# Lcressot/fhe-string-bounty

Measured on AMD Instinct MI355X. Metric: PBS/sec (whole node), higher is better.
Workload: dtype f64

## Files before the change

### fhe-string-bounty_amd/csrc/engine.h

```cpp
#pragma once
#include <hip/hip_runtime.h>
#include <stdint.h>

#include <map>
#include <mutex>
#include <string>
#include <vector>

#include "../../include/fhestr.h"

#define FHESTR_KERNEL_REVISION "r04.2"

namespace fhe {

inline uint32_t n_ggsw(const fhe_params_t& p) {
    return p.grouping_factor > 1 ? p.n / p.grouping_factor * (1u << p.grouping_factor) : p.n;
}
inline uint64_t multi_bit_key_bit(const uint64_t* group_bits, uint32_t g, uint32_t sel) {
    uint64_t prod = 1;
    for (uint32_t b = 0; b < g; b++) prod *= group_bits[b] ^ (((sel >> (g - 1 - b)) & 1) ^ 1);
    return prod;
}

void aes128_round_keys(const uint8_t key[16], uint8_t rk[11][16]);
const uint8_t* aes_sbox();

extern thread_local std::string g_last_error;
int fail(const std::string& msg);

struct BrVariant;

uint64_t fill_accumulator(const fhe_params_t& p, const uint64_t* table, std::vector<uint64_t>& acc);
void fill_accumulator_torus(const fhe_params_t& p, const uint64_t* box_values, std::vector<uint64_t>& acc);

struct EngineEnv {
    int log2_points = 0;
    int wide_fair = -1;
    int keep_busy = -1;
    int overlap_streams = -1;
    int ks_mfma = -1;
    int ks_chunks = -1;
    int cluster_mode = -2;
    int cluster_spin_limit = -1;
    int multibit_combine_max = -1;
    int cluster_test_fault = -1;
    int dense_per_cu = -1;
    int cluster_fallback = -1;
    static EngineEnv read();
};

struct Engine {
    std::recursive_mutex mu;
    fhe_params_t p{};
    int device = 0;
    hipStream_t stream = nullptr;
    hipStream_t own_stream = nullptr;
    std::map<std::vector<uint64_t>, uint32_t> lut_dedup;
    hipEvent_t ev[3] = {nullptr, nullptr, nullptr};
    std::vector<hipEvent_t> ring;
    size_t ring_used = 0;
    const BrVariant* variant = nullptr;
    const BrVariant* variant_large = nullptr;
    int cu_count = 256;
    int pipeline = 0;
    hipStream_t ks_stream = nullptr;
    hipEvent_t pipe_ev[5] = {nullptr, nullptr, nullptr, nullptr, nullptr};
    hipEvent_t pipe_input_ready = nullptr;
    const void* pipe_out[2] = {nullptr, nullptr};
    size_t pipe_out_bytes[2] = {0, 0};
    static constexpr int OVL_MAX = 4;
    int ovl_streams = 2;
    uint32_t wide_fair_shift = 13;
    uint32_t dense_per_cu = 2;
    bool keep_busy = false;
    hipStream_t ovl_stream[OVL_MAX] = {nullptr, nullptr, nullptr, nullptr};
    hipEvent_t ovl_done[OVL_MAX] = {nullptr, nullptr, nullptr, nullptr};
    struct ByteRange { const char* lo; const char* hi; };
    std::vector<ByteRange> ovl_ins[OVL_MAX], ovl_outs[OVL_MAX];
    uint64_t* ovl_small[OVL_MAX] = {nullptr, nullptr, nullptr, nullptr};
    size_t ovl_cap_small[OVL_MAX] = {0, 0, 0, 0};
    int8_t* ovl_digits[OVL_MAX] = {nullptr, nullptr, nullptr, nullptr};
    size_t ovl_cap_digits[OVL_MAX] = {0, 0, 0, 0};
    int sync_all_streams();
    void end_pipeline_run();
    uint64_t pipe_calls = 0;
    int shadow_fit = -1;
    uint32_t multibit_combine_max = 64;

    uint32_t* d_ksk_packed = nullptr;
    uint64_t* d_ksk_rowsum = nullptr;
    int8_t* d_ksk_mfma = nullptr;
    int8_t* d_ks_digits = nullptr;
    size_t cap_ks_digits = 0;
    bool ks_mfma_enabled = true;
    double* d_fbsk = nullptr;
    double* d_fbsk_dense = nullptr;
    uint64_t* d_luts = nullptr;
    size_t luts_cap = 0;
    uint32_t n_luts = 0;

    uint64_t *d_in = nullptr, *d_small = nullptr, *d_small2 = nullptr, *d_out = nullptr, *d_pool = nullptr;
    uint32_t* d_idx = nullptr;
    uint32_t* d_slot_exp = nullptr;
    size_t multibit_workspace_cap = 0;
    void* d_meta = nullptr;
    uint64_t* d_compact = nullptr;
    size_t cap_compact = 0;
    void* d_ws = nullptr;
    size_t cap_ws = 0;
    void* d_cluster_ws = nullptr;
    size_t cap_cluster_ws = 0;
    void* d_cluster_ctl = nullptr;
    bool cluster_unchecked = false;
    uint32_t cluster_last = 0;
    bool cluster_fallback = true;
    uint32_t cluster_fallbacks = 0;
    uint32_t cluster_last_error = 0;
    int cluster_mode = -1;
    uint32_t cluster_max_batch = 0xFFFFFFFFu;
    uint32_t ks_chunks_override = 0;
    int xcd_per_cu = -1;
    uint32_t xcd_auto_max = 16;
    uint32_t cluster_spin_limit = 1u << 22;
    uint32_t cluster_test_fault = 0;
    int cluster_check();
    size_t cap_in = 0, cap_small = 0, cap_small2 = 0, cap_out = 0, cap_idx = 0, cap_pool = 0, cap_meta = 0;

    static int create(const fhe_params_t& p, int device, Engine** out);
    ~Engine();
    int use();
    int set_variant(int logR);
    int allow_rotate_lds();
    int load_keys(const uint64_t* bsk_std, const uint64_t* ksk);
    int load_seeded_keys(const uint8_t ksk_seed[16], const uint64_t* ksk_bodies, const uint8_t bsk_seed[16], const uint64_t* bsk_bodies,
                         uint64_t* bsk_std_out, uint64_t* ksk_out);
    int expand_seeded_lwe(const uint8_t* seeds, const uint64_t* bodies, uint32_t count, uint64_t* d_out, uint64_t* host_out);
    int expand_compact_list(const uint64_t* list, uint32_t count, uint64_t* d_out, uint64_t* host_out);
    int expand_compact_list_dev(const uint64_t* d_list, uint32_t count, uint64_t* d_out);
    int generate_keys(const uint64_t* glwe_sk, const uint64_t* small_sk, const uint8_t seed[32],
                      uint64_t* bsk_std_out, uint64_t* ksk_out);
    int install_keys(uint64_t* d_ksk_std, uint64_t* d_bsk_std);
    int convert_polys(const uint64_t* d_std, double* d_out, uint32_t n_polys);
    int cluster_settle(const uint64_t* d_sm, const uint32_t* d_lut_idx, uint64_t* d_big, uint32_t count);
    int probe_slot_exponents();
    uint64_t fill_accumulator(const uint64_t* table, std::vector<uint64_t>& acc) const { return fhe::fill_accumulator(p, table, acc); }
    int lut_upload_dedup(const std::vector<uint64_t>& acc, uint32_t* id);
    int set_stream(hipStream_t s, bool use_own);
    int lut_upload(const uint64_t* acc, uint32_t* id);
    int lut_download(uint32_t id, uint64_t* acc);
    int ensure_batch(uint32_t count);
    int check_lut_idx(const uint32_t* lut_idx, uint32_t count) const;

    int launch_keyswitch(const uint64_t* d_big, uint64_t* d_sm, uint32_t count, hipStream_t on = nullptr, bool shadow = false, int digits_slot = 0);
    int launch_blind_rotate(const uint64_t* d_sm, const uint32_t* d_lut_idx, uint64_t* d_big, uint32_t count, hipStream_t on = nullptr, bool two_per_cu = false,
                            bool one_workgroup_only = false);
    bool shadow_keyswitch_fits();
    int ks_pbs_dev(const uint64_t* d_big_in, const uint32_t* d_lut_idx, uint64_t* d_big_out, uint32_t count, bool allow_pipeline = false);
    int ks_pbs_host(const uint64_t* in, const uint32_t* lut_idx, uint64_t* out, uint32_t count);
    int keyswitch_host(const uint64_t* in, uint64_t* out_small, uint32_t count);
    int pbs_host(const uint64_t* in_small, const uint32_t* lut_idx, uint64_t* out, uint32_t count);
    int pbs_ks_host(const uint64_t* in_small, const uint32_t* lut_idx, uint64_t* out_small, uint32_t count);
    int lincomb_dev(const uint64_t* d_pool, const uint32_t* d_off, const uint32_t* d_src,
                    const int32_t* d_coeff, const uint64_t* d_cst, uint64_t* d_out, uint32_t jobs);
// ... 26 lines not shown
```

### fhe-string-bounty_amd/csrc/engine.hip

```cpp
#include "engine.h"

#include <algorithm>
#include <cmath>
#include <cstdio>
#include <cstdlib>
#include <cstring>
#include <string>

#include "keygen_kernels.hip.h"
#include "lwe_kernels.hip.h"
#include "ks_mfma_kernels.hip.h"
#include "pbs_kernels.hip.h"
#include "pbs_dense_kernels.hip.h"
#include "pbs_large_kernels.hip.h"
#include "pbs_cluster_kernels.hip.h"
#include "pbs_xcd_kernels.hip.h"
#include "pbs_multibit_kernels.hip.h"
#include "pbs_seq_kernels.hip.h"
#include "seeded_kernels.hip.h"
#include "compact_kernels.hip.h"

namespace fhe {

thread_local std::string g_last_error;
// ... 166 lines not shown
                                  : reinterpret_cast<const void*>(&multibit_combine_generic_kernel<3>);
    v.combined_bytes = (size_t)v.L * v.k1 * v.k1 * ((size_t)1 << (v.logN - 1)) * 16;
    return v;
}
template <int LOGN, int LOGR, int K1, int L>
BrVariant make_multibit_generic_variant(int G) {
    return make_multibit_two_kernel_variant<&blind_rotate_kernel<LOGN, LOGR, K1, L, true>>(make_variant<LOGN, LOGR, K1, L>(), G);
}
template <int LOGN, int K1, int L>
BrVariant make_multibit_seq_variant(int G) {
    return make_multibit_two_kernel_variant<&blind_rotate_seq_kernel<LOGN, K1, L, true>>(make_seq_variant<LOGN, K1, L>(), G);
}

static const std::vector<BrVariant>& variants() {
    static const std::vector<BrVariant> v = {
        make_variant<11, 2, 2, 1>(), make_variant<11, 3, 2, 1>(), make_variant<11, 4, 2, 1>(),
        make_wide_variant<11, 2, 2, 1>(), make_wide_variant<11, 3, 2, 1>(),
        make_multibit_variant<11, 2, 2, 2>(),
        make_multibit_variant<11, 2, 2, 3>(),
        make_multibit_generic_variant<9, 2, 4, 1>(2), make_multibit_generic_variant<9, 2, 4, 1>(3),
        make_multibit_seq_variant<13, 2, 2>(2), make_multibit_seq_variant<13, 2, 2>(3),
        make_multibit_generic_variant<8, 2, 2, 2>(2), make_multibit_generic_variant<8, 2, 2, 2>(3),
        make_multibit_generic_variant<7, 2, 3, 1>(2), make_multibit_generic_variant<7, 2, 3, 1>(3),
        make_variant<10, 2, 3, 1>(), make_variant<10, 3, 3, 1>(), make_wide_variant<10, 2, 3, 1>(),
        make_variant<9, 2, 4, 1>(),
        make_variant<8, 2, 2, 2>(), make_variant<7, 2, 3, 1>(),
        make_wide_variant<8, 2, 2, 2>(), make_wide_variant<7, 2, 3, 1>(),
        make_variant<8, 2, 6, 1>(),
        make_variant<9, 2, 3, 2>(),
        make_wide_variant<12, 2, 2, 1>(), make_wide_variant<12, 2, 2, 2>(),
        make_seq_variant<13, 2, 1>(), make_seq_variant<13, 2, 2>(),
        make_large_variant<14, 2, 2>(),
        make_large_variant<15, 2, 2>(),
        make_large_variant<14, 2, 3>(), make_large_variant<15, 2, 3>(),
    };
    return v;
}

static const BrVariant* find_variant(const fhe_params_t& p, int selector) {
    int logN = 0;
    while ((1u << logN) < p.N) logN++;
    const int logR = selector & 15;
    const bool wide = (selector & 16) != 0;
    const int grouping = p.grouping_factor > 1 ? (int)p.grouping_factor : 1;
    for (const auto& v : variants())
        if (v.logN == logN && v.k1 == (int)p.k + 1 && v.L == (int)p.pbs_level && v.grouping == grouping &&
            (selector == 0 || (v.logR == logR && v.wide == wide)))
            return &v;
    return nullptr;
}

struct BrVariantPair { const BrVariant *small, *large; };
static BrVariantPair find_variant_pair(const fhe_params_t& p, int selector) {
    const BrVariant* v = find_variant(p, selector);
    const BrVariant* w = v && selector == 0 ? find_variant(p, v->logR | 16) : nullptr;
    return {v, w ? w : v};
}

static size_t rotate_lds(const BrVariant* v, const fhe_params_t& p) { return v->lds_bytes + (size_t)p.n * v->lds_per_n; }

int params_supported(const fhe_params_t& p, int selector) {
    if ((p.N & (p.N - 1)) || p.N < 128) return fail("polynomial size must be a power of two >= 128");
    if (p.pbs_base_log < 1 || p.pbs_base_log > 31 || p.pbs_base_log * p.pbs_level > (p.pbs_level >= 3 ? 62u : 31u))
        return fail("unsupported PBS decomposition (base_log * level must be <= 31, or <= 62 with >= 3 levels)");
    if (p.ks_level < 1 || p.ks_base_log < 1 || p.ks_base_log > 7 || p.ks_base_log * p.ks_level > 62)
        return fail("unsupported keyswitch decomposition (base_log 1..7, base_log * level <= 62)");
    if (p.msg_mod * p.carry_mod == 0 || (p.N % (p.msg_mod * p.carry_mod)) != 0)
        return fail("msg_mod * carry_mod must divide N");
    if (p.grouping_factor > 1 && (p.n % p.grouping_factor) != 0) return fail("grouping factor must divide n");
    if (!find_variant(p, selector)) return fail("no blind-rotation kernel instantiated for this (N, k, level, grouping factor)");
    return 0;
}
int params_supported(const fhe_params_t& p) { return params_supported(p, 0); }

EngineEnv EngineEnv::read() {
    EngineEnv v;
    auto num = [](const char* name, int& out) { if (const char* t = getenv(name)) out = atoi(t); };
    num("FHESTR_LOG2_POINTS", v.log2_points);
    num("FHESTR_WIDE_FAIR", v.wide_fair);
    num("FHESTR_DENSE_PER_CU", v.dense_per_cu);
    num("FHESTR_CLUSTER_FALLBACK", v.cluster_fallback);
    num("FHESTR_KEEP_BUSY", v.keep_busy);
    num("FHESTR_OVERLAP_STREAMS", v.overlap_streams);
    num("FHESTR_KS_MFMA", v.ks_mfma);
    num("FHESTR_KS_CHUNKS", v.ks_chunks);
    num("FHESTR_CLUSTER", v.cluster_mode);
    num("FHESTR_CLUSTER_SPIN_LIMIT", v.cluster_spin_limit);
    num("FHESTR_MULTIBIT_COMBINE_MAX", v.multibit_combine_max);
    num("FHESTR_CLUSTER_TEST_FAULT", v.cluster_test_fault);
    return v;
}

int Engine::create(const fhe_params_t& p, int device, Engine** out) {
    const EngineEnv env = EngineEnv::read();
    if (params_supported(p, env.log2_points)) return 1;
    int count = 0;
    HIP_TRY(hipGetDeviceCount(&count));
    if (count <= 0) return fail("no HIP device: libfhestr has no CPU fallback");
    if (device < 0 || device >= count) return fail("bad device index");
    HIP_TRY(hipSetDevice(device));
    Engine* e = new Engine();
    e->p = p;
    e->device = device;
    const BrVariantPair vp = find_variant_pair(p, env.log2_points);
    e->variant = vp.small;
    e->variant_large = vp.large;
    if (env.wide_fair >= 0) e->wide_fair_shift = (uint32_t)std::min(20, env.wide_fair);
    if (env.dense_per_cu >= 0) e->dense_per_cu = (uint32_t)env.dense_per_cu;
    if (env.cluster_fallback >= 0) e->cluster_fallback = env.cluster_fallback != 0;
    if (env.keep_busy >= 0) e->keep_busy = env.keep_busy != 0;
    if (env.overlap_streams >= 0) e->ovl_streams = std::min((int)Engine::OVL_MAX, std::max(2, env.overlap_streams));
    if (env.ks_mfma >= 0) e->ks_mfma_enabled = env.ks_mfma != 0;
    if (env.ks_chunks >= 0) e->ks_chunks_override = (uint32_t)env.ks_chunks;
    if (env.cluster_spin_limit >= 0) e->cluster_spin_limit = (uint32_t)std::max(64, env.cluster_spin_limit);
    if (env.cluster_mode > -2) e->cluster_mode = std::min(2, std::max(-1, env.cluster_mode));
    if (env.multibit_combine_max >= 0) e->multibit_combine_max = (uint32_t)std::min(1024, env.multibit_combine_max);
#ifdef FHESTR_TEST_HOOKS
    if (env.cluster_test_fault >= 0) e->cluster_test_fault = (uint32_t)env.cluster_test_fault;
#endif
    hipDeviceProp_t prop;
    HIP_TRY(hipGetDeviceProperties(&prop, device));
    e->cu_count = prop.multiProcessorCount;
    HIP_TRY(hipStreamCreateWithFlags(&e->own_stream, hipStreamNonBlocking));
    e->stream = e->own_stream;
    for (auto& ev : e->ev) HIP_TRY(hipEventCreate(&ev));
    *out = e;
    return 0;
}

Engine::~Engine() {
    (void)hipSetDevice(device);
    if (stream) (void)sync_all_streams();
    auto rel = [](void* ptr) { if (ptr) (void)hipFree(ptr); };
    rel(d_ksk_packed); rel(d_ksk_rowsum); rel(d_fbsk); rel(d_fbsk_dense); rel(d_luts); rel(d_in); rel(d_small); rel(d_small2); rel(d_out); rel(d_idx);
    rel(d_pool); rel(d_meta); rel(d_ws); rel(d_slot_exp); rel(d_cluster_ws); rel(d_cluster_ctl); rel(d_ksk_mfma); rel(d_ks_digits); rel(d_compact);
    for (int q = 0; q < OVL_MAX; q++) { rel(ovl_digits[q]); rel(ovl_small[q]); if (ovl_done[q]) (void)hipEventDestroy(ovl_done[q]); if (q >= 2 && ovl_stream[q]) (void)hipStreamDestroy(ovl_stream[q]); }
    for (auto& e : ev) if (e) (void)hipEventDestroy(e);
    for (auto& e : ring) if (e) (void)hipEventDestroy(e);
    for (auto& e : pipe_ev) if (e) (void)hipEventDestroy(e);
    if (ks_stream) (void)hipStreamDestroy(ks_stream);
    if (own_stream) (void)hipStreamDestroy(own_stream);
}

int Engine::set_stream(hipStream_t s, bool use_own) {
    if (use()) return 1;
    if (ks_stream) HIP_TRY(hipStreamSynchronize(ks_stream));
    HIP_TRY(hipStreamSynchronize(stream));
    stream = use_own ? own_stream : s;
    return 0;
}

int Engine::lut_upload_dedup(const std::vector<uint64_t>& acc, uint32_t* id) {
    auto it = lut_dedup.find(acc);
    if (it != lut_dedup.end()) { *id = it->second; return 0; }
    if (lut_upload(acc.data(), id)) return 1;
    lut_dedup[acc] = *id;
    return 0;
}

int Engine::use() { HIP_TRY(hipSetDevice(device)); return 0; }

static int ensure(void** ptr, size_t* cap, size_t bytes) {
    if (*cap >= bytes) return 0;
    if (*ptr) HIP_TRY(hipFree(*ptr));
    *ptr = nullptr; *cap = 0;
    HIP_TRY(hipMalloc(ptr, bytes));
    *cap = bytes;
    return 0;
}

int Engine::set_variant(int logR) {
    const BrVariantPair vp = find_variant_pair(p, logR);
    if (!vp.small) return fail("no such blind-rotation variant for these parameters");
    if (d_fbsk && vp.small->logR != variant->logR)
        return fail("variant must be chosen before fhe_engine_load_keys (Fourier key layout depends on it)");
    variant = vp.small;
    variant_large = vp.large;
    shadow_fit = -1;
    return d_fbsk ? allow_rotate_lds() : 0;
}

int Engine::allow_rotate_lds() {
    HIP_TRY(hipFuncSetAttribute(variant->rotate_fn, hipFuncAttributeMaxDynamicSharedMemorySize, (int)rotate_lds(variant, p)));
    HIP_TRY(hipFuncSetAttribute(variant_large->rotate_fn, hipFuncAttributeMaxDynamicSharedMemorySize, (int)rotate_lds(variant_large, p)));
    if (variant->rotate_combined_fn)
        HIP_TRY(hipFuncSetAttribute(variant->rotate_combined_fn, hipFuncAttributeMaxDynamicSharedMemorySize, (int)rotate_lds(variant, p)));
    return 0;
}

int Engine::load_keys(const uint64_t* bsk_std, const uint64_t* ksk) {
    if (use()) return 1;
    const size_t ksk_len = (size_t)p.k * p.N * p.ks_level * (p.n + 1);
    const size_t bsk_len = (size_t)n_ggsw(p) * p.pbs_level * (p.k + 1) * (p.k + 1) * p.N;
    uint64_t *d_ksk_std = nullptr, *d_bsk_std = nullptr;
    HIP_TRY(hipMalloc((void**)&d_ksk_std, ksk_len * 8));
    if (hipMalloc((void**)&d_bsk_std, bsk_len * 8) != hipSuccess) {
        (void)hipFree(d_ksk_std);
        return fail("hipMalloc of the standard-domain bootstrap key failed");
    }
    hipError_t e = hipMemcpyAsync(d_ksk_std, ksk, ksk_len * 8, hipMemcpyHostToDevice, stream);
    if (e == hipSuccess) e = hipMemcpyAsync(d_bsk_std, bsk_std, bsk_len * 8, hipMemcpyHostToDevice, stream);
    if (e != hipSuccess) {
        (void)hipFree(d_ksk_std); (void)hipFree(d_bsk_std);
        return fail(std::string("key upload: ") + hipGetErrorString(e));
    }
    return install_keys(d_ksk_std, d_bsk_std);
}

int Engine::load_seeded_keys(const uint8_t ksk_seed[16], const uint64_t* ksk_bodies, const uint8_t bsk_seed[16],
                             const uint64_t* bsk_bodies, uint64_t* bsk_std_out, uint64_t* ksk_out) {
    if (use()) return 1;
    const uint64_t ksk_rows = (uint64_t)p.k * p.N * p.ks_level, bsk_rows = (uint64_t)n_ggsw(p) * p.pbs_level * (p.k + 1);
    const size_t ksk_len = ksk_rows * (p.n + 1), bsk_len = bsk_rows * (p.k + 1) * p.N;
    const size_t bsk_body_words = bsk_rows * p.N;
    uint64_t *d_ksk_std = nullptr, *d_bsk_std = nullptr, *d_bodies = nullptr;
    uint8_t* d_sbox = nullptr;
    auto cleanup = [&] { (void)hipFree(d_ksk_std); (void)hipFree(d_bsk_std); (void)hipFree(d_bodies); (void)hipFree(d_sbox); };
    hipError_t e = hipMalloc((void**)&d_ksk_std, ksk_len * 8);
    if (e == hipSuccess) e = hipMalloc((void**)&d_bsk_std, bsk_len * 8);
    if (e == hipSuccess) e = hipMalloc((void**)&d_bodies, (bsk_body_words + ksk_rows) * 8);
    if (e == hipSuccess) e = hipMalloc((void**)&d_sbox, 256);
    if (e == hipSuccess) e = hipMemcpyAsync(d_sbox, aes_sbox(), 256, hipMemcpyHostToDevice, stream);
    if (e == hipSuccess) e = hipMemcpyAsync(d_bodies, bsk_bodies, bsk_body_words * 8, hipMemcpyHostToDevice, stream);
    if (e == hipSuccess) e = hipMemcpyAsync(d_bodies + bsk_body_words, ksk_bodies, ksk_rows * 8, hipMemcpyHostToDevice, stream);
    if (e != hipSuccess) { cleanup(); return fail(std::string("load_seeded_keys: ") + hipGetErrorString(e)); }
    SeededExpandArgs ka{}, ba{};
    aes128_round_keys(ksk_seed, ka.round_keys);
    ka.out = d_ksk_std; ka.rows = ksk_rows; ka.mask_per_row = p.n; ka.row_words = p.n + 1;
    aes128_round_keys(bsk_seed, ba.round_keys);
// ... 460 lines not shown
    return 0;
}

static int rotate_dense(Engine& e, const BrVariant* v, BlindRotateArgs a) {
    a.fair_shift = 0;
    a.fbsk = e.d_fbsk_dense;
    void* args[] = {(void*)&a};
    HIP_TRY(hipLaunchKernel(v->dense_fn, dim3(a.batch), dim3(v->threads), args, v->dense_lds + (size_t)e.p.n * v->lds_per_n, e.stream));
    return 0;
}

static int rotate_plain(Engine& e, const BrVariant* v, BlindRotateArgs a) {
    uint32_t grid = a.batch;
    if (e.keep_busy && !v->wide && !v->large && a.batch * 2 <= (uint32_t)e.cu_count) grid = a.batch * ((uint32_t)e.cu_count / a.batch);
    if (!(a.fbsk = rotation_key(e, v))) return fail("wide kernel: the key copy in its plan's order is missing");
    void* args[] = {(void*)&a};
    HIP_TRY(hipLaunchKernel(v->rotate_keypf_fn && v->wide ? v->rotate_keypf_fn : v->rotate_fn, dim3(grid), dim3(v->threads), args,
                            rotate_lds(v, e.p), e.stream));
    return 0;
}

int Engine::launch_blind_rotate(const uint64_t* d_sm, const uint32_t* d_lut_idx, uint64_t* d_big, uint32_t count, hipStream_t on,
                                bool two_per_cu, bool one_workgroup_only) {
    if (!d_fbsk) return fail("keys not loaded");
    if (n_luts == 0) return fail("no lookup table uploaded");
    BlindRotateArgs a{d_sm, d_lut_idx, d_luts, d_fbsk, d_big, p.n, p.pbs_base_log, count};
    a.grouping = 0;
    const uint32_t cus = (uint32_t)cu_count;
    a.fair_shift = (count > cus && (((count + cus - 1) / cus) & 1u) == 0) ? wide_fair_shift : 0u;
    const BrVariant* v = nullptr;
    switch (choose_rotate_path(*this, count, two_per_cu, one_workgroup_only, v)) {
        case BrPath::Overlapped: return rotate_overlapped(*this, v, a, on ? on : stream);
        case BrPath::MultiBitCombined: return rotate_multibit_combined(*this, v, a);
        case BrPath::MultiBitTwoKernel: return rotate_multibit_two_kernel(*this, v, a);
        case BrPath::WholeXcd: return rotate_whole_xcd(*this, v, a);
        case BrPath::Cluster:
            return rotate_multi_cu(*this, a, v->cluster_fn, (uint32_t)v->cluster_size, v->threads, v->cluster_lds + (size_t)p.n * 4, 0, v->cluster_ws, 1);
        case BrPath::Large: return rotate_large(*this, v, a);
        case BrPath::Dense: return rotate_dense(*this, v, a);
        case BrPath::Plain: break;
    }
    return rotate_plain(*this, v, a);
}

bool Engine::shadow_keyswitch_fits() {
    if (shadow_fit < 0) {
        hipFuncAttributes fa{};
        shadow_fit = 0;
        if (hipFuncGetAttributes(&fa, variant->rotate_fn) == hipSuccess) {
            const int waves_per_simd = (variant->threads / 64 + 3) / 4;
            const int regs = (fa.numRegs + 7) / 8 * 8;
            shadow_fit = waves_per_simd * regs + 64 <= 512 ? 1 : 0;
        }
    }
    return shadow_fit == 1;
}

int Engine::ks_pbs_dev(const uint64_t* d_big_in, const uint32_t* d_lut_idx, uint64_t* d_big_out,
                       uint32_t count, bool allow_pipeline) {
    if (use()) return 1;
    if (count == 0) return 0;
    const size_t small = (size_t)p.n + 1;
    if (ensure((void**)&d_small, &cap_small, count * small * 8)) return 1;
    constexpr size_t RING = 1024;
    if (ring.empty()) {
        ring.resize(RING * 4);
        for (auto& e : ring) HIP_TRY(hipEventCreate(&e));
    }
    hipEvent_t* e4 = &ring[(ring_used % RING) * 4];
    ring_used++;
    if (allow_pipeline && pipeline == 2 && overlapped_mode_eligible(*this, count)) {
        const int ns = ovl_streams;
        if (!ks_stream) {
            HIP_TRY(hipStreamCreateWithFlags(&ks_stream, hipStreamNonBlocking));
            for (auto& e : pipe_ev) HIP_TRY(hipEventCreateWithFlags(&e, hipEventDisableTiming));
        }
        for (int q = 2; q < ns; q++)
            if (!ovl_stream[q]) {
                HIP_TRY(hipStreamCreateWithFlags(&ovl_stream[q], hipStreamNonBlocking));
                HIP_TRY(hipEventCreateWithFlags(&ovl_done[q], hipEventDisableTiming));
            }
        for (int q = 0; q < 2; q++)
            if (!ovl_done[q]) HIP_TRY(hipEventCreateWithFlags(&ovl_done[q], hipEventDisableTiming));
        const int slot = (int)(pipe_calls % (uint64_t)ns);
        hipStream_t s = slot == 0 ? stream : slot == 1 ? ks_stream : ovl_stream[slot];
        if (ensure((void**)&ovl_small[slot], &ovl_cap_small[slot], count * small * 8)) return 1;
        uint64_t* sm = ovl_small[slot];
        const size_t big = (size_t)p.k * p.N + 1;
        const char *in_lo = (const char*)d_big_in, *in_hi = in_lo + (size_t)count * big * 8;
        const char *out_lo = (const char*)d_big_out, *out_hi = out_lo + (size_t)count * big * 8;
        if (pipe_calls == 0) HIP_TRY(hipEventRecord(pipe_ev[4], stream));
        if (pipe_calls < (uint64_t)ns && slot != 0) HIP_TRY(hipStreamWaitEvent(s, pipe_ev[4], 0));
        if (pipe_input_ready) {
            HIP_TRY(hipStreamWaitEvent(s, pipe_input_ready, 0));
            pipe_input_ready = nullptr;
        }
        auto overlaps = [](const char* a_lo, const char* a_hi, const std::vector<ByteRange>& rs) {
            for (const auto& r : rs)
                if (a_lo < r.hi && r.lo < a_hi) return true;
            return false;
        };
        for (int q = 0; q < ns; q++) {
            if (q == slot || !ovl_done[q] || (ovl_ins[q].empty() && ovl_outs[q].empty())) continue;
            if (overlaps(in_lo, in_hi, ovl_outs[q]) || overlaps(out_lo, out_hi, ovl_outs[q]) || overlaps(out_lo, out_hi, ovl_ins[q]))
                HIP_TRY(hipStreamWaitEvent(s, ovl_done[q], 0));
        }
        auto remember = [](std::vector<ByteRange>& rs, const char* lo, const char* hi) {
            for (auto& r : rs)
                if (r.lo == lo && r.hi == hi) return;
            if (rs.size() < 32) { rs.push_back({lo, hi}); return; }
            rs[0].lo = std::min(rs[0].lo, lo);
            rs[0].hi = std::max(rs[0].hi, hi);
        };
        remember(ovl_ins[slot], in_lo, in_hi);
        remember(ovl_outs[slot], out_lo, out_hi);
        HIP_TRY(hipEventRecord(e4[0], s));
        if (launch_keyswitch(d_big_in, sm, count, s, false, slot)) return 1;
        HIP_TRY(hipEventRecord(e4[1], s));
        HIP_TRY(hipEventRecord(e4[2], s));
        if (launch_blind_rotate(sm, d_lut_idx, d_big_out, count, s, true)) return 1;
        HIP_TRY(hipEventRecord(e4[3], s));
        HIP_TRY(hipEventRecord(ovl_done[slot], s));
        pipe_calls++;
        return 0;
    }
    if (allow_pipeline && pipeline == 1 && shadow_mode_eligible(*this, count) && shadow_keyswitch_fits()) {
        if (!ks_stream) {
            HIP_TRY(hipStreamCreateWithFlags(&ks_stream, hipStreamNonBlocking));
            for (auto& e : pipe_ev) HIP_TRY(hipEventCreateWithFlags(&e, hipEventDisableTiming));
        }
        if (ensure((void**)&d_small2, &cap_small2, count * small * 8)) return 1;
        const int slot = (int)(pipe_calls & 1);
        uint64_t* sm = slot ? d_small2 : d_small;
        const size_t big = (size_t)p.k * p.N + 1;
        const char *in_lo = (const char*)d_big_in, *in_hi = in_lo + (size_t)count * big * 8;
        const char* prev = (const char*)pipe_out[slot ^ 1];
        if (pipe_calls == 0) {
            HIP_TRY(hipEventRecord(pipe_ev[4], stream));
            HIP_TRY(hipStreamWaitEvent(ks_stream, pipe_ev[4], 0));
        }
        if (pipe_input_ready) {
            HIP_TRY(hipStreamWaitEvent(ks_stream, pipe_input_ready, 0));
            pipe_input_ready = nullptr;
        }
        if (pipe_calls >= 1 && prev && in_lo < prev + pipe_out_bytes[slot ^ 1] && prev < in_hi)
            HIP_TRY(hipStreamWaitEvent(ks_stream, pipe_ev[2 + (slot ^ 1)], 0));
        if (pipe_calls >= 2) HIP_TRY(hipStreamWaitEvent(ks_stream, pipe_ev[2 + slot], 0));
        HIP_TRY(hipEventRecord(e4[0], ks_stream));
        if (launch_keyswitch(d_big_in, sm, count, ks_stream, true)) return 1;
        HIP_TRY(hipEventRecord(e4[1], ks_stream));
        HIP_TRY(hipEventRecord(pipe_ev[slot], ks_stream));
        HIP_TRY(hipStreamWaitEvent(stream, pipe_ev[slot], 0));
        HIP_TRY(hipEventRecord(e4[2], stream));
        if (launch_blind_rotate(sm, d_lut_idx, d_big_out, count)) return 1;
        HIP_TRY(hipEventRecord(e4[3], stream));
        HIP_TRY(hipEventRecord(pipe_ev[2 + slot], stream));
        pipe_out[slot] = d_big_out;
        pipe_out_bytes[slot] = (size_t)count * big * 8;
        pipe_calls++;
        return 0;
    }
    if (ks_stream && pipe_calls) {
        HIP_TRY(hipStreamSynchronize(ks_stream));
        for (int q = 2; q < OVL_MAX; q++) if (ovl_stream[q]) HIP_TRY(hipStreamSynchronize(ovl_stream[q]));
        end_pipeline_run();
    }
    pipe_input_ready = nullptr;
    HIP_TRY(hipEventRecord(e4[0], stream));
    if (launch_keyswitch(d_big_in, d_small, count)) return 1;
    HIP_TRY(hipEventRecord(e4[1], stream));
    HIP_TRY(hipEventRecord(e4[2], stream));
    if (launch_blind_rotate(d_small, d_lut_idx, d_big_out, count)) return 1;
    HIP_TRY(hipEventRecord(e4[3], stream));
    return 0;
}

int Engine::check_lut_idx(const uint32_t* lut_idx, uint32_t count) const {
    if (n_luts == 0) return fail("no lookup table uploaded");
    if (lut_idx)
        for (uint32_t i = 0; i < count; i++)
            if (lut_idx[i] >= n_luts) return fail("lut_idx out of range");
    return 0;
}

int Engine::ks_pbs_host(const uint64_t* in, const uint32_t* lut_idx, uint64_t* out, uint32_t count) {
    if (use()) return 1;
    if (count == 0) return 0;
    if (check_lut_idx(lut_idx, count)) return 1;
    if (ensure_batch(count)) return 1;
    const size_t big = (size_t)p.k * p.N + 1;
    HIP_TRY(hipMemcpyAsync(d_in, in, count * big * 8, hipMemcpyHostToDevice, stream));
    if (lut_idx) HIP_TRY(hipMemcpyAsync(d_idx, lut_idx, (size_t)count * 4, hipMemcpyHostToDevice, stream));
    if (ks_pbs_dev(d_in, lut_idx ? d_idx : nullptr, d_out, count)) return 1;
    HIP_TRY(hipMemcpyAsync(out, d_out, count * big * 8, hipMemcpyDeviceToHost, stream));
    HIP_TRY(hipStreamSynchronize(stream));
    return cluster_check();
}

int Engine::keyswitch_host(const uint64_t* in, uint64_t* out_small, uint32_t count) {
    if (use()) return 1;
    if (count == 0) return 0;
    if (ensure_batch(count)) return 1;
    const size_t big = (size_t)p.k * p.N + 1, small = (size_t)p.n + 1;
    HIP_TRY(hipMemcpyAsync(d_in, in, count * big * 8, hipMemcpyHostToDevice, stream));
    if (launch_keyswitch(d_in, d_small, count)) return 1;
    HIP_TRY(hipMemcpyAsync(out_small, d_small, count * small * 8, hipMemcpyDeviceToHost, stream));
    HIP_TRY(hipStreamSynchronize(stream));
    return 0;
}

int Engine::pbs_host(const uint64_t* in_small, const uint32_t* lut_idx, uint64_t* out, uint32_t count) {
    if (use()) return 1;
    if (count == 0) return 0;
    if (check_lut_idx(lut_idx, count)) return 1;
    if (ensure_batch(count)) return 1;
    const size_t big = (size_t)p.k * p.N + 1, small = (size_t)p.n + 1;
    HIP_TRY(hipMemcpyAsync(d_small, in_small, count * small * 8, hipMemcpyHostToDevice, stream));
    if (lut_idx) HIP_TRY(hipMemcpyAsync(d_idx, lut_idx, (size_t)count * 4, hipMemcpyHostToDevice, stream));
    if (launch_blind_rotate(d_small, lut_idx ? d_idx : nullptr, d_out, count)) return 1;
    HIP_TRY(hipMemcpyAsync(out, d_out, count * big * 8, hipMemcpyDeviceToHost, stream));
    HIP_TRY(hipStreamSynchronize(stream));
    return cluster_check();
}

int Engine::pbs_ks_host(const uint64_t* in_small, const uint32_t* lut_idx, uint64_t* out_small, uint32_t count) {
    if (use()) return 1;
    if (count == 0) return 0;
    if (check_lut_idx(lut_idx, count)) return 1;
    if (ensure_batch(count)) return 1;
    const size_t small = (size_t)p.n + 1;
    if (ensure((void**)&d_small2, &cap_small2, count * small * 8)) return 1;
    HIP_TRY(hipMemcpyAsync(d_small, in_small, count * small * 8, hipMemcpyHostToDevice, stream));
    if (lut_idx) HIP_TRY(hipMemcpyAsync(d_idx, lut_idx, (size_t)count * 4, hipMemcpyHostToDevice, stream));
    if (launch_blind_rotate(d_small, lut_idx ? d_idx : nullptr, d_out, count)) return 1;
    if (launch_keyswitch(d_out, d_small2, count)) return 1;
    HIP_TRY(hipMemcpyAsync(out_small, d_small2, count * small * 8, hipMemcpyDeviceToHost, stream));
    HIP_TRY(hipStreamSynchronize(stream));
    return cluster_check();
}

int Engine::lincomb_dev(const uint64_t* d_pool_, const uint32_t* d_off, const uint32_t* d_src,
                        const int32_t* d_coeff, const uint64_t* d_cst, uint64_t* d_o, uint32_t jobs) {
    if (jobs == 0) return 0;
    LincombArgs a{d_pool_, d_off, d_src, d_coeff, d_cst, d_o, p.k * p.N + 1, jobs};
    hipLaunchKernelGGL(lincomb_kernel, dim3(jobs), dim3(256), 0, stream, a);
    HIP_TRY(hipGetLastError());
// ... 19 lines not shown
                       out_slot, out_inst);
    HIP_TRY(hipGetLastError());
    return 0;
}

int Engine::lincomb_host(const uint64_t* pool, uint32_t pool_count, const uint32_t* off,
                         const uint32_t* src, const int32_t* coeff, const uint64_t* cst,
                         uint64_t* out, uint32_t jobs) {
    if (use()) return 1;
    if (jobs == 0) return 0;
    const size_t big = (size_t)p.k * p.N + 1;
    const uint32_t terms = off[jobs];
    for (uint32_t t = 0; t < terms; t++)
        if (src[t] >= pool_count) return fail("lincomb source index out of range");
    if (ensure((void**)&d_pool, &cap_pool, (size_t)pool_count * big * 8)) return 1;
    if (ensure((void**)&d_out, &cap_out, (size_t)jobs * big * 8)) return 1;
    const size_t o_off = 0, o_src = o_off + ((size_t)(jobs + 1) * 4 + 7) / 8 * 8;
    const size_t o_coeff = o_src + ((size_t)terms * 4 + 7) / 8 * 8;
    const size_t o_cst = o_coeff + ((size_t)terms * 4 + 7) / 8 * 8;
    const size_t meta_bytes = o_cst + (size_t)jobs * 8;
    if (ensure((void**)&d_meta, &cap_meta, meta_bytes)) return 1;
    unsigned char* m = reinterpret_cast<unsigned char*>(d_meta);
    HIP_TRY(hipMemcpyAsync(d_pool, pool, (size_t)pool_count * big * 8, hipMemcpyHostToDevice, stream));
    HIP_TRY(hipMemcpyAsync(m + o_off, off, (size_t)(jobs + 1) * 4, hipMemcpyHostToDevice, stream));
    HIP_TRY(hipMemcpyAsync(m + o_src, src, (size_t)terms * 4, hipMemcpyHostToDevice, stream));
    HIP_TRY(hipMemcpyAsync(m + o_coeff, coeff, (size_t)terms * 4, hipMemcpyHostToDevice, stream));
    HIP_TRY(hipMemcpyAsync(m + o_cst, cst, (size_t)jobs * 8, hipMemcpyHostToDevice, stream));
    if (lincomb_dev(d_pool, (const uint32_t*)(m + o_off), (const uint32_t*)(m + o_src),
                    (const int32_t*)(m + o_coeff), (const uint64_t*)(m + o_cst), d_out, jobs))
        return 1;
    HIP_TRY(hipMemcpyAsync(out, d_out, (size_t)jobs * big * 8, hipMemcpyDeviceToHost, stream));
    HIP_TRY(hipStreamSynchronize(stream));
    return 0;
}

int Engine::last_kernel_ms(float ms[2]) {
    if (use()) return 1;
    if (ring_used == 0) return fail("no ks_pbs call recorded");
    hipEvent_t* e4 = &ring[((ring_used - 1) % 1024) * 4];
    if (sync_all_streams()) return 1;
    HIP_TRY(hipEventSynchronize(e4[3]));
    HIP_TRY(hipEventElapsedTime(&ms[0], e4[0], e4[1]));
    HIP_TRY(hipEventElapsedTime(&ms[1], e4[2], e4[3]));
    return 0;
}

int Engine::kernel_times(double total_ms[2], uint32_t* calls, bool reset) {
    if (use()) return 1;
    if (sync_all_streams()) return 1;
    const size_t nrec = ring_used < 1024 ? ring_used : 1024;
    total_ms[0] = total_ms[1] = 0.0;
    for (size_t c = 0; c < nrec; c++) {
        hipEvent_t* e4 = &ring[((ring_used - 1 - c) % 1024) * 4];
        float a = 0, b = 0;
        HIP_TRY(hipEventElapsedTime(&a, e4[0], e4[1]));
        HIP_TRY(hipEventElapsedTime(&b, e4[2], e4[3]));
        total_ms[0] += a;
        total_ms[1] += b;
    }
    *calls = (uint32_t)nrec;
    if (reset) ring_used = 0;
    return 0;
}

#ifdef FHESTR_WALL
extern "C" int fhe_debug_read_wall(unsigned long long* out, size_t count) {
    return hipMemcpyFromSymbol(out, HIP_SYMBOL(g_wall), count * sizeof(unsigned long long), 0, hipMemcpyDeviceToHost) == hipSuccess ? 0 : 1;
}
#endif
#ifdef FHESTR_STAMPS
extern "C" int fhe_debug_read_stamps(unsigned long long* out, size_t count) {
    return hipMemcpyFromSymbol(out, HIP_SYMBOL(g_stamps), count * sizeof(unsigned long long), 0, hipMemcpyDeviceToHost) == hipSuccess ? 0 : 1;
}
#endif

int Engine::synchronize() {
    if (use()) return 1;
    if (sync_all_streams()) return 1;
    end_pipeline_run();
    return cluster_check();
}

int Engine::sync_all_streams() {
    if (ks_stream) HIP_TRY(hipStreamSynchronize(ks_stream));
    for (int q = 2; q < OVL_MAX; q++) if (ovl_stream[q]) HIP_TRY(hipStreamSynchronize(ovl_stream[q]));
    HIP_TRY(hipStreamSynchronize(stream));
    return 0;
}

void Engine::end_pipeline_run() {
    pipe_calls = 0;
    pipe_out[0] = pipe_out[1] = nullptr;
    for (int q = 0; q < OVL_MAX; q++) { ovl_ins[q].clear(); ovl_outs[q].clear(); }
}

int Engine::cluster_settle(const uint64_t* d_sm, const uint32_t* d_lut_idx, uint64_t* d_big, uint32_t count) {
    if (!cluster_fallback) { cluster_unchecked = true; return 0; }
    ClusterStatus st{};
    ClusterStatus* d_st = reinterpret_cast<ClusterStatus*>(reinterpret_cast<ClusterCtl*>(d_cluster_ctl) + 1);
    HIP_TRY(hipMemcpyAsync(&st, d_st, sizeof(st), hipMemcpyDeviceToHost, stream));
    HIP_TRY(hipStreamSynchronize(stream));
    cluster_last = st.clusters;
    if (!st.error) return 0;
    HIP_TRY(hipMemsetAsync(d_st, 0, sizeof(st), stream));
    cluster_fallbacks++;
    cluster_last_error = st.error;
    return launch_blind_rotate(d_sm, d_lut_idx, d_big, count, nullptr, false, true);
}

int Engine::cluster_check() {
    if (!cluster_unchecked || !d_cluster_ctl) return 0;
    ClusterStatus st{};
    HIP_TRY(hipMemcpy(&st, reinterpret_cast<ClusterCtl*>(d_cluster_ctl) + 1, sizeof(st), hipMemcpyDeviceToHost));
    cluster_unchecked = false;
    cluster_last = st.clusters;
    if (st.error) {
        HIP_TRY(hipMemset(reinterpret_cast<ClusterCtl*>(d_cluster_ctl) + 1, 0, sizeof(st)));
        return fail("blind_rotate_cluster_kernel: a cluster hand-over timed out (code " + std::to_string(st.error) +
                    "); results of that launch are invalid");
    }
    return 0;
}

}
```

Measured before the change: 125,400.

## Run overlapped keyswitches ahead on a dedicated stream with double-buffered outputs

In the multi-stream overlap path, keyswitch now runs on a separate dedicated stream rather than each slot's blind-rotate stream. Each slot gets two small-ciphertext buffers, with read events that guard reuse. This lets the next batch's keyswitch proceed while earlier blind rotates are still running, hiding keyswitch latency. The cost is extra buffers, events and cross-stream waits, and all keyswitches now share one digits slot, which could serialize them or contend for it.

New measurement: 88720. 29.3% lower.

```diff
diff --git a/fhe-string-bounty_amd/csrc/engine.h b/fhe-string-bounty_amd/csrc/engine.h
--- a/fhe-string-bounty_amd/csrc/engine.h
+++ b/fhe-string-bounty_amd/csrc/engine.h
@@ -38,6 +38,7 @@
     int wide_fair = -1;
     int keep_busy = -1;
     int overlap_streams = -1;
+    int ks_ahead = -1;
     int ks_mfma = -1;
     int ks_chunks = -1;
     int cluster_mode = -2;
@@ -77,8 +78,11 @@
     hipEvent_t ovl_done[OVL_MAX] = {nullptr, nullptr, nullptr, nullptr};
     struct ByteRange { const char* lo; const char* hi; };
     std::vector<ByteRange> ovl_ins[OVL_MAX], ovl_outs[OVL_MAX];
-    uint64_t* ovl_small[OVL_MAX] = {nullptr, nullptr, nullptr, nullptr};
-    size_t ovl_cap_small[OVL_MAX] = {0, 0, 0, 0};
+    bool ks_ahead = true;
+    hipStream_t ovl_ks_stream = nullptr;
+    uint64_t* ovl_small[2 * OVL_MAX] = {};
+    size_t ovl_cap_small[2 * OVL_MAX] = {};
+    hipEvent_t ovl_read[2 * OVL_MAX] = {};
     int8_t* ovl_digits[OVL_MAX] = {nullptr, nullptr, nullptr, nullptr};
     size_t ovl_cap_digits[OVL_MAX] = {0, 0, 0, 0};
     int sync_all_streams();
diff --git a/fhe-string-bounty_amd/csrc/engine.hip b/fhe-string-bounty_amd/csrc/engine.hip
--- a/fhe-string-bounty_amd/csrc/engine.hip
+++ b/fhe-string-bounty_amd/csrc/engine.hip
@@ -272,6 +272,7 @@
     num("FHESTR_CLUSTER_FALLBACK", v.cluster_fallback);
     num("FHESTR_KEEP_BUSY", v.keep_busy);
     num("FHESTR_OVERLAP_STREAMS", v.overlap_streams);
+    num("FHESTR_KS_AHEAD", v.ks_ahead);
     num("FHESTR_KS_MFMA", v.ks_mfma);
     num("FHESTR_KS_CHUNKS", v.ks_chunks);
     num("FHESTR_CLUSTER", v.cluster_mode);
@@ -300,6 +301,7 @@
     if (env.cluster_fallback >= 0) e->cluster_fallback = env.cluster_fallback != 0;
     if (env.keep_busy >= 0) e->keep_busy = env.keep_busy != 0;
     if (env.overlap_streams >= 0) e->ovl_streams = std::min((int)Engine::OVL_MAX, std::max(2, env.overlap_streams));
+    if (env.ks_ahead >= 0) e->ks_ahead = env.ks_ahead != 0;
     if (env.ks_mfma >= 0) e->ks_mfma_enabled = env.ks_mfma != 0;
     if (env.ks_chunks >= 0) e->ks_chunks_override = (uint32_t)env.ks_chunks;
     if (env.cluster_spin_limit >= 0) e->cluster_spin_limit = (uint32_t)std::max(64, env.cluster_spin_limit);
@@ -324,7 +326,9 @@
     auto rel = [](void* ptr) { if (ptr) (void)hipFree(ptr); };
     rel(d_ksk_packed); rel(d_ksk_rowsum); rel(d_fbsk); rel(d_fbsk_dense); rel(d_luts); rel(d_in); rel(d_small); rel(d_small2); rel(d_out); rel(d_idx);
     rel(d_pool); rel(d_meta); rel(d_ws); rel(d_slot_exp); rel(d_cluster_ws); rel(d_cluster_ctl); rel(d_ksk_mfma); rel(d_ks_digits); rel(d_compact);
-    for (int q = 0; q < OVL_MAX; q++) { rel(ovl_digits[q]); rel(ovl_small[q]); if (ovl_done[q]) (void)hipEventDestroy(ovl_done[q]); if (q >= 2 && ovl_stream[q]) (void)hipStreamDestroy(ovl_stream[q]); }
+    for (int b = 0; b < 2 * OVL_MAX; b++) { rel(ovl_small[b]); if (ovl_read[b]) (void)hipEventDestroy(ovl_read[b]); }
+    if (ovl_ks_stream) (void)hipStreamDestroy(ovl_ks_stream);
+    for (int q = 0; q < OVL_MAX; q++) { rel(ovl_digits[q]); if (ovl_done[q]) (void)hipEventDestroy(ovl_done[q]); if (q >= 2 && ovl_stream[q]) (void)hipStreamDestroy(ovl_stream[q]); }
     for (auto& e : ev) if (e) (void)hipEventDestroy(e);
     for (auto& e : ring) if (e) (void)hipEventDestroy(e);
     for (auto& e : pipe_ev) if (e) (void)hipEventDestroy(e);
@@ -335,6 +339,7 @@
 int Engine::set_stream(hipStream_t s, bool use_own) {
     if (use()) return 1;
     if (ks_stream) HIP_TRY(hipStreamSynchronize(ks_stream));
+    if (ovl_ks_stream) HIP_TRY(hipStreamSynchronize(ovl_ks_stream));
     HIP_TRY(hipStreamSynchronize(stream));
     stream = use_own ? own_stream : s;
     return 0;
@@ -961,27 +966,37 @@
             }
         for (int q = 0; q < 2; q++)
             if (!ovl_done[q]) HIP_TRY(hipEventCreateWithFlags(&ovl_done[q], hipEventDisableTiming));
+        const bool ahead = ks_ahead && ns < OVL_MAX;
+        if (ahead && !ovl_ks_stream) HIP_TRY(hipStreamCreateWithFlags(&ovl_ks_stream, hipStreamNonBlocking));
         const int slot = (int)(pipe_calls % (uint64_t)ns);
+        const int buf = 2 * slot + (int)((pipe_calls / (uint64_t)ns) & 1);
         hipStream_t s = slot == 0 ? stream : slot == 1 ? ks_stream : ovl_stream[slot];
-        if (ensure((void**)&ovl_small[slot], &ovl_cap_small[slot], count * small * 8)) return 1;
-        uint64_t* sm = ovl_small[slot];
+        hipStream_t k = ahead ? ovl_ks_stream : s;
+        if (ensure((void**)&ovl_small[buf], &ovl_cap_small[buf], count * small * 8)) return 1;
+        if (!ovl_read[buf]) HIP_TRY(hipEventCreateWithFlags(&ovl_read[buf], hipEventDisableTiming));
+        uint64_t* sm = ovl_small[buf];
         const size_t big = (size_t)p.k * p.N + 1;
         const char *in_lo = (const char*)d_big_in, *in_hi = in_lo + (size_t)count * big * 8;
         const char *out_lo = (const char*)d_big_out, *out_hi = out_lo + (size_t)count * big * 8;
         if (pipe_calls == 0) HIP_TRY(hipEventRecord(pipe_ev[4], stream));
-        if (pipe_calls < (uint64_t)ns && slot != 0) HIP_TRY(hipStreamWaitEvent(s, pipe_ev[4], 0));
+        if (pipe_calls < (uint64_t)ns) {
+            if (slot != 0) HIP_TRY(hipStreamWaitEvent(s, pipe_ev[4], 0));
+            if (k != s) HIP_TRY(hipStreamWaitEvent(k, pipe_ev[4], 0));
+        }
         if (pipe_input_ready) {
-            HIP_TRY(hipStreamWaitEvent(s, pipe_input_ready, 0));
+            HIP_TRY(hipStreamWaitEvent(k, pipe_input_ready, 0));
             pipe_input_ready = nullptr;
         }
+        if (k != s && pipe_calls >= 2 * (uint64_t)ns) HIP_TRY(hipStreamWaitEvent(k, ovl_read[buf], 0));
         auto overlaps = [](const char* a_lo, const char* a_hi, const std::vector<ByteRange>& rs) {
             for (const auto& r : rs)
                 if (a_lo < r.hi && r.lo < a_hi) return true;
             return false;
         };
         for (int q = 0; q < ns; q++) {
-            if (q == slot || !ovl_done[q] || (ovl_ins[q].empty() && ovl_outs[q].empty())) continue;
-            if (overlaps(in_lo, in_hi, ovl_outs[q]) || overlaps(out_lo, out_hi, ovl_outs[q]) || overlaps(out_lo, out_hi, ovl_ins[q]))
+            if (!ovl_done[q] || (ovl_ins[q].empty() && ovl_outs[q].empty())) continue;
+            if ((q != slot || k != s) && overlaps(in_lo, in_hi, ovl_outs[q])) HIP_TRY(hipStreamWaitEvent(k, ovl_done[q], 0));
+            if (q != slot && (overlaps(out_lo, out_hi, ovl_outs[q]) || overlaps(out_lo, out_hi, ovl_ins[q])))
                 HIP_TRY(hipStreamWaitEvent(s, ovl_done[q], 0));
         }
         auto remember = [](std::vector<ByteRange>& rs, const char* lo, const char* hi) {
@@ -993,13 +1008,15 @@
         };
         remember(ovl_ins[slot], in_lo, in_hi);
         remember(ovl_outs[slot], out_lo, out_hi);
-        HIP_TRY(hipEventRecord(e4[0], s));
-        if (launch_keyswitch(d_big_in, sm, count, s, false, slot)) return 1;
-        HIP_TRY(hipEventRecord(e4[1], s));
+        HIP_TRY(hipEventRecord(e4[0], k));
+        if (launch_keyswitch(d_big_in, sm, count, k, false, ahead ? 1 : slot)) return 1;
+        HIP_TRY(hipEventRecord(e4[1], k));
+        if (k != s) HIP_TRY(hipStreamWaitEvent(s, e4[1], 0));
         HIP_TRY(hipEventRecord(e4[2], s));
         if (launch_blind_rotate(sm, d_lut_idx, d_big_out, count, s, true)) return 1;
         HIP_TRY(hipEventRecord(e4[3], s));
         HIP_TRY(hipEventRecord(ovl_done[slot], s));
+        HIP_TRY(hipEventRecord(ovl_read[buf], s));
         pipe_calls++;
         return 0;
     }
@@ -1041,6 +1058,7 @@
     }
     if (ks_stream && pipe_calls) {
         HIP_TRY(hipStreamSynchronize(ks_stream));
+        if (ovl_ks_stream) HIP_TRY(hipStreamSynchronize(ovl_ks_stream));
         for (int q = 2; q < OVL_MAX; q++) if (ovl_stream[q]) HIP_TRY(hipStreamSynchronize(ovl_stream[q]));
         end_pipeline_run();
     }
@@ -1226,6 +1244,7 @@
 }
 
 int Engine::sync_all_streams() {
+    if (ovl_ks_stream) HIP_TRY(hipStreamSynchronize(ovl_ks_stream));
     if (ks_stream) HIP_TRY(hipStreamSynchronize(ks_stream));
     for (int q = 2; q < OVL_MAX; q++) if (ovl_stream[q]) HIP_TRY(hipStreamSynchronize(ovl_stream[q]));
     HIP_TRY(hipStreamSynchronize(stream));
```
